# sayands/sgaligner

Measured on AMD Instinct MI355X. Metric: subscan-pairs/sec (fwd+bwd) + node-match Hits@1 vs reference, higher is better.
Workload: dtype f32 (fp32 operands and fp32 accumulation throughout; the anchors x negatives loss sweeps multiply them as three exact bf16 planes, six bf16 MFMAs per product...

## Files before the change

include/sgaligner_hip.h:

```cpp
#ifndef SGALIGNER_HIP_H
#define SGALIGNER_HIP_H
#include <stddef.h>
#include <stdint.h>
#ifdef __cplusplus
extern "C" {
#endif

int sga_version(void);
const char* sga_last_error(void);
int sga_device_cus(void);

int sga_pointnet_fwd(const float* x, const float* w1, const float* b1, const float* w2, const float* b2,
                     const float* w3, const float* b3, float* y, int32_t* argmax, int T, int P, int C3,
                     void* stream);
size_t sga_pointnet_fwd_ws_bytes(int T, int C3);
int sga_pointnet_fwd_ws(const float* x, const float* w1, const float* b1, const float* w2, const float* b2,
                        const float* w3, const float* b3, float* y, int32_t* argmax, int T, int P, int C3,
                        void* workspace, size_t ws_bytes, int mode, void* stream);
size_t sga_pointnet_fwd_bn_ws_bytes(int T, int C3);
int sga_pointnet_fwd_bn(const float* x, const float* w1, const float* b1, const float* w2, const float* b2,
                        const float* w3, const float* b3, float* y, int32_t* argmax, int T, int P, int C3,
                        void* workspace, size_t ws_bytes, void* bn_workspace, size_t bn_ws_bytes, double* bn_sums, int mode, void* stream);
int sga_pointnet_bwd(const float* x, const int32_t* argmax, const float* y, const float* gy, const float* w1,
                     const float* b1, const float* w2, const float* b2, const float* w3, float* gw1, float* gb1,
// ... 71 lines not shown
                      float* dZ, void* stream);
int sga_loss_neg_sums_shard(const float* Z, int Dp, int A, int J1, int J2, float tau0, float tau1, double* sums8, int a_lo, int a_hi,
                            void* stream);
int sga_loss_neg_grad_shard(const float* Z, int Dp, int A, int J1, int J2, float tau0, float tau1, const double* gs8,
                            float* dZ, int a_lo, int a_hi, void* stream);
size_t sga_loss_anchor_f16_ws_bytes(int NT, int A, int ns);
int sga_loss_anchor_fwd_f16(const float* const* Z, const void* const* Zh, const int* Dp, int NT, int A, const double* sums,
                            float alpha, float tau_icl, float tau_ial, double* out, int a_lo, int a_hi, void* ws, size_t ws_bytes,
                            void* stream);
int sga_loss_anchor_bwd_f16(const float* const* Z, const void* const* Zh, const int* Dp, int NT, int A, const double* sums,
                            float alpha, float tau_icl, float tau_ial, const float* coef, float* const* M1,
                            double* gs, int a_lo, int a_hi, void* ws, size_t ws_bytes, void* stream);

int sga_loss_stash_grad(const float* M1, const float* Z, int A, int Dp, float* dZ, int a_lo, int a_hi, void* stream);
int sga_loss_multi_sums(const float* const* Z, int M, int D, const float* beta, int A, int J1, int J2, float tau0, float tau1,
                        double* sums, int a_lo, int a_hi, void* stream);
int sga_loss_multi_grad(const float* const* Z, int M, int D, const float* beta, int A, int J1, int J2, float tau0, float tau1,
                        const double* gs, float* const* dZ, double* gamma, int a_lo, int a_hi, void* stream);
size_t sga_loss_centre_bytes(void);
int sga_loss_centre_tables(const float* Z, int A, int J1, int J2, float* Zc, void* stat_ws, void* stream);
int sga_loss_multi_sums_centred(const float* const* Zc, int M, const float* beta, int A, int J1, int J2, float tau0, float tau1,
                                double* sums, int a_lo, int a_hi, void* stream);
int sga_loss_multi_grad_centred(const float* const* Zc, int M, const float* beta, int A, int J1, int J2, float tau0, float tau1,
                                const double* gs, float* const* dZ, double* gamma, int a_lo, int a_hi, void* stream);
int sga_loss_scatter_tangent_stat(const float* dZ, const float* Z, const float* nrm, const int32_t* idx, int R, int D,
                                  const void* stat_ws, float* dE, void* stream);
int sga_loss_anchor_multi_fwd(const float* const* Z, int M, const float* beta, int A, const double* sums, float alpha,
                              float tau_icl, float tau_ial, double* out, int a_lo, int a_hi, void* stream);
int sga_loss_anchor_multi_bwd(const float* const* Z, int M, const float* beta, int A, const double* sums, float alpha,
                              float tau_icl, float tau_ial, const float* coef, float* const* M1, double* gs, double* gamma,
                              int a_lo, int a_hi, double* out_terms, void* stream);
int sga_loss_anchor_multi_bwd_symx(const float* const* Z, int M, const float* beta, int A, const double* sums, float alpha,
                                   float tau_icl, float tau_ial, const float* coef, float* const* M1, float* const* M2,
                                   double* gs, double* gamma, int a_lo, int a_hi, int j_lo, int j_hi, int mir, double* out_terms, void* stream);
int sga_loss_stash_grad_symx(const float* M1, const float* M2, const float* Z, int A, int Dp, float* dZ, int a_lo, int a_hi,
                             int j_lo, int j_hi, int mir, void* stream);

int sga_loss_check_norms(const float* nrm, int n, float* poison, void* stream);

size_t sga_loss_split3_bytes(int A, int J1, int J2);
int sga_loss_split3_tables(const float* Z, int A, int J1, int J2, void* Zb, float* Zc, void* stream);
int sga_loss_multi_sums_bf16x6(const void* const* Zb, int M, const float* beta, int A, int J1, int J2, float tau0, float tau1,
                               double* sums, int a_lo, int a_hi, int lite, void* stream);
int sga_loss_multi_grad_bf16x6(const void* const* Zb, int M, const float* beta, int A, int J1, int J2, float tau0, float tau1,
                               const double* gs, float* const* dZ, double* gamma, int a_lo, int a_hi, void* stream);
int sga_loss_scatter_tangent(const float* dZ, const float* Z, const float* nrm, const int32_t* idx, int A, int J1, int J2, int D,
                             const void* Zb, float* dE, void* stream);
int sga_loss_stash_grad_symx_bf16x6(const float* M1, const float* M2, const void* Zb, int A, int J1, int J2, float* dZ,
                                    int a_lo, int a_hi, int j_lo, int j_hi, int mir, void* stream);
int sga_loss_anchor_multi_bwd_symx_bf16x6(const void* const* Zb, int M, const float* beta, int A, int J1, int J2, const double* sums,
                                          float alpha, float tau_icl, float tau_ial, const float* coef, float* const* M1, float* const* M2,
                                          double* gs, double* gamma, int a_lo, int a_hi, int j_lo, int j_hi, int mir, double* out_terms,
                                          void* stream);

int sga_group_loss_fwd(const float* const* Z, int M, const float* beta, int A, int J1, const int32_t* groups, int G,
                       const int64_t* s_off, int64_t s_total, float alpha, float tau_icl, float tau_ial, float* S,
                       double* sums, double* out, int use_valu, void* stream);
int sga_group_loss_bwd(const float* const* Z, int M, const float* beta, int A, int J1, const int32_t* groups, int G,
                       const int64_t* s_off, int64_t s_total, float alpha, float tau_icl, float tau_ial, float* S,
                       const double* sums, const float* coef, float* const* dZ, double* gamma, int use_valu, void* stream);

size_t sga_simrank_workspace_bytes(int T);
size_t sga_simrank_workspace_bytes_f16(int T, int D);
int sga_simrank(const float* E, int T, int D, const int32_t* pair_off, const int32_t* blk_pair, const int32_t* blk_row, int n_blocks, int B,
                int max_pair_objects, const int32_t* q_idx, const int32_t* q_tgt, int Q, int K, int32_t* rank,
                int32_t* topk_idx, float* topk_sim, int f16, void* workspace, size_t workspace_bytes, void* stream);
int sga_pair_metrics(const int32_t* rank, const int32_t* topk_idx, const float* topk_sim, int K, const int32_t* q_tgt,
                     const int32_t* pair_off, const int32_t* pair_q_off, int B, float* out, void* stream);

int sga_gemm_ex(int transA, int transB, int M, int N, int K, const float* A, long lda, const float* B, long ldb,
                float* C, long ldc, const float* bias, int act, const float* resid, long ldr, void* stream);
int sga_pct_attention(const float* Q, long ldq, const float* V, long ldv, int T, int N, float* stats, float* Xs,
                      long ldx, void* stream);
int sga_pct_attention_bwd(const float* Q, long ldq, const float* V, long ldv, const float* dXs, long ldd, int T, int N,
                          const float* stats, float* work, float* dQ, long ldo, float* dV, long ldw, void* stream);
int sga_segment_max(const float* Y, long ldy, int T, int N, int C, float* G, int32_t* argmax, void* stream);
int sga_segment_max_bwd(const float* dG, const int32_t* argmax, int T, int N, int C, float* dY, long ldd, void* stream);
int sga_pct_head_prep(const float* dG, const float* G, const float* gamma, const float* beta, const float* fin, int T, int C, long R,
                      int training, float slope, float* coef, float* ab, void* stream);
int sga_pct_head_dw(const float* WG, const float* W, const float* ab, const float* cs, const float* coef, const int32_t* amax,
                    const float* cat, long ldc, int T, int N, int C, int K, float* dW, float* Wb, float* a0, void* stream);
int sga_pct_head_scatter(const float* coef, const int32_t* amax, const float* W, int T, int N, int C, int K, float* dcat, long ldd,
                         void* stream);
int sga_segment_max_affine(const float* Y, long ldy, int T, int N, int C, const float* scale, const float* shift, float slope, float* G,
                           int32_t* argmax, void* stream);

int sga_bn_stats(const float* X, long ldx, int R, int C, double* sums, void* stream);
int sga_bn_finalize(const double* sums, int R, int C, const float* gamma, const float* beta, float* running_mean, float* running_var,
                    long long* num_batches_tracked, float momentum, float eps, int training, float* out, void* stream);
int sga_bn_bwd_finalize(const double* sums, int R, int C, float* out, void* stream);
int sga_bn_apply(const float* X, long ldx, int R, int C, const float* scale, const float* shift, int act,
                 const float* resid, long ldr, float* Y, long ldy, void* stream);
int sga_bn_bwd_stats(const float* X, long ldx, const float* dY, long ldd, int R, int C, const float* scale,
                     const float* shift, const float* mean, const float* rstd, int act, double* sums, void* stream);
int sga_bn_bwd_apply(const float* X, long ldx, const float* dY, long ldd, int R, int C, const float* scale,
                     const float* shift, const float* mean, const float* rstd, const float* mean_g,
                     const float* mean_gx, int act, float* dX, long ldo, void* stream);

size_t sga_fps_scratch_floats(int total_points);
int sga_fps(const float* pts, const int32_t* offsets, int n_obj, const int32_t* start, int npoint,
            const int32_t* work_small, int n_small, const int32_t* work_mid, int n_mid,
            const int32_t* work_large, int n_large, int32_t* out_idx, float* scratch, void* stream);

int sga_hull_candidates(const float* pts, const int32_t* offsets, int n_obj, unsigned char* keep, int32_t* n_planes, void* stream);
int sga_hull_max_candidates(void);
int sga_hull_vertices(const double* pts, const int32_t* offsets, int n_obj, unsigned char* is_vertex, int32_t* status, void* stream);
// ... 70 lines not shown
```

sgaligner_amd/_lib.py:

```python
from __future__ import annotations

import ctypes
import os
from ctypes import c_char_p, c_double, c_float, c_int, c_int64, c_long, c_size_t, c_void_p

_HERE = os.path.dirname(os.path.abspath(__file__))
LIB_PATH = os.environ.get('SGA_LIB_PATH') or os.path.join(_HERE, 'csrc', 'libsga_hip.so')
_lib = None

P = c_void_p
I = c_int
F = c_float

SIGNATURES = {
    'sga_version': (I, []),
    'sga_last_error': (c_char_p, []),
    'sga_device_cus': (I, []),
    'sga_pointnet_fwd': (I, [P, P, P, P, P, P, P, P, P, I, I, I, P]),
    'sga_pointnet_fwd_ws_bytes': (c_size_t, [I, I]),
    'sga_loss_neg_grad_wide_floats': (c_size_t, [I, I, I]),
    'sga_loss_neg_grad_wide': (I, [P, I, I, I, I, c_float, c_float, P, P, P, c_size_t, P]),
    'sga_wide16_ldt': (c_long, [I, I, I]),
    'sga_wide16_prepare': (I, [P, I, I, I, I, P, P, P]),
    'sga_loss_neg_sums_f16': (I, [P, I, I, I, I, c_float, c_float, P, I, I, P]),
# ... 38 lines not shown
    'sga_hull_max_candidates': (I, []),
    'sga_hull_vertices': (I, [P, P, I, P, P, P]),
    'sga_nn_workspace_bytes': (c_size_t, [I, I, I]),
    'sga_nn_search': (I, [P, P, I, I, P, I, P, I, I, I, I, P, P, I, P, P, P, c_size_t, P]),
    'sga_ransac_workspace_bytes': (c_size_t, [I, I, I, I]),
    'sga_ransac_rigid': (I, [P, P, I, I, P, P, I, I, I, I, P, P, c_double, I, P, P, P, P, P, P, P, c_size_t, P]),
    'sga_subscan_lds_slots': (I, []),
    'sga_frame_visibility': (I, [P, P, P, P, P, P, I, I, I, c_int64, I, I, P, P, P, P, P]),
    'sga_subscan_walk': (I, [P, P, P, P, P, P, I, I, I, c_int64, P, P, P, P, P, P, P, P]),
    'sga_subscan_object_counts': (I, [P, P, P, P, I, I, I, c_int64, I, P, I, P, I, P, P, P, P, P, P]),
    'sga_scenegraph_lds_slots': (I, []),
    'sga_scenegraph_tile': (I, []),
    'sga_graph_max_nodes': (I, []),
    'sga_object_counts': (I, [P, P, P, I, I, I, I, P, P, P, P]),
    'sga_object_partition_ws_bytes': (c_size_t, [I, I, I]),
    'sga_object_partition': (I, [P, P, P, P, P, I, I, I, I, I, I, P, P, P, P, P, P, P, c_size_t, P]),
    'sga_graph_complete': (I, [P, P, P, P, I, P, P, I, I, P, P, P, P, P, P, P, P, P, P]),
    'sga_bow_counts': (I, [P, P, I, I, I, P, P, P, P]),
    'sga_gemm': (I, [I, I, I, I, I, P, c_long, I, P, c_long, P, c_long, P, I, P]),
    'sga_colsum': (I, [P, c_long, I, I, P, I, P]),
    'sga_gemm_bnstats': (I, [I, I, I, P, c_long, P, c_long, P, c_long, P, P, P]),
    'sga_cast_f64_f32': (I, [P, P, c_size_t, P]),
    'sga_gemm_plan': (I, [I, I, I, I, I, c_long, c_long, c_long, c_long] + [I] * 9 + [P, P, P]),
    'sga_loss_gather': (I, [P, I, I, P, I, P, I, P, P]),
    'sga_loss_scatter': (I, [P, P, P, P, I, I, I, P, P]),
    'sga_loss_neg_sums': (I, [P, I, I, I, I, F, F, P, P]),
    'sga_loss_neg_grad': (I, [P, I, I, I, I, F, F, P, P, P]),
    'sga_loss_neg_sums_shard': (I, [P, I, I, I, I, F, F, P, I, I, P]),
    'sga_loss_neg_grad_shard': (I, [P, I, I, I, I, F, F, P, P, I, I, P]),
    'sga_loss_anchor_f16_ws_bytes': (c_size_t, [I, I, I]),
    'sga_loss_anchor_fwd_f16': (I, [P, P, P, I, I, P, F, F, F, P, I, I, P, c_size_t, P]),
    'sga_loss_anchor_bwd_f16': (I, [P, P, P, I, I, P, F, F, F, P, P, P, I, I, P, c_size_t, P]),
    'sga_loss_stash_grad_f16_bytes': (c_size_t, [I, I]),
    'sga_loss_stash_grad_f16': (I, [P, P, I, I, I, I, P, I, I, P, c_size_t, P]),
    'sga_loss_multi_sums': (I, [P, I, I, P, I, I, I, F, F, P, I, I, P]),
    'sga_loss_multi_grad': (I, [P, I, I, P, I, I, I, F, F, P, P, P, I, I, P]),
    'sga_loss_centre_bytes': (c_size_t, []),
    'sga_loss_centre_tables': (I, [P, I, I, I, P, P, P]),
    'sga_loss_multi_sums_centred': (I, [P, I, P, I, I, I, F, F, P, I, I, P]),
    'sga_loss_multi_grad_centred': (I, [P, I, P, I, I, I, F, F, P, P, P, I, I, P]),
    'sga_loss_scatter_tangent_stat': (I, [P, P, P, P, I, I, P, P, P]),
    'sga_loss_check_norms': (I, [P, I, P, P]),
    'sga_loss_slots': (I, []),
    'sga_loss_anchor_multi_fwd': (I, [P, I, P, I, P, F, F, F, P, I, I, P]),
    'sga_loss_anchor_multi_bwd': (I, [P, I, P, I, P, F, F, F, P, P, P, P, I, I, P, P]),
    'sga_loss_stash_grad': (I, [P, P, I, I, P, I, I, P]),
    'sga_loss_anchor_multi_bwd_symx': (I, [P, I, P, I, P, F, F, F, P, P, P, P, P, I, I, I, I, I, P, P]),
    'sga_loss_stash_grad_symx': (I, [P, P, P, I, I, P, I, I, I, I, I, P]),
    'sga_loss_split3_bytes': (c_size_t, [I, I, I]),
    'sga_loss_split3_tables': (I, [P, I, I, I, P, P, P]),
    'sga_loss_scatter_tangent': (I, [P, P, P, P, I, I, I, I, P, P, P]),
    'sga_loss_stash_grad_symx_bf16x6': (I, [P, P, P, I, I, I, P, I, I, I, I, I, P]),
    'sga_loss_anchor_multi_bwd_symx_bf16x6': (I, [P, I, P, I, I, I, P, F, F, F, P, P, P, P, P, I, I, I, I, I, P, P]),
    'sga_loss_multi_sums_bf16x6': (I, [P, I, P, I, I, I, F, F, P, I, I, I, P]),
    'sga_loss_multi_grad_bf16x6': (I, [P, I, P, I, I, I, F, F, P, P, P, I, I, P]),
    'sga_group_loss_fwd': (I, [P, I, P, I, I, P, I, P, c_int64, F, F, F, P, P, P, I, P]),
    'sga_group_loss_bwd': (I, [P, I, P, I, I, P, I, P, c_int64, F, F, F, P, P, P, P, P, I, P]),
    'sga_fusion_fwd': (I, [P, I, P, P, I, I, P]),
    'sga_fusion_bwd_workspace_bytes': (c_size_t, [I]),
    'sga_fusion_bwd': (I, [P, I, P, P, P, P, I, I, P, c_size_t, P]),
    'sga_fusion_var_fwd': (I, [P, I, P, P, P, I, P]),
    'sga_fusion_var_bwd': (I, [P, I, P, P, P, P, P, I, P, c_size_t, P]),
    'sga_gcn_aggregate': (I, [P, I, P, P, P, P, I, I, I, I, P, P, P]),
    'sga_relu_bwd': (I, [P, P, P, c_size_t, P]),
    'sga_nca_row_group': (I, []),
    'sga_nca_block_sums': (I, [P, c_long, I, I, I, F, F, P, P, P, P]),
    'sga_nca_loss': (I, [P, P, I, P, I, F, F, P, P, P, P, P]),
    'sga_nca_coef': (I, [P, c_long, P, c_long, P, c_long, I, I, I, F, F, F, P, P, P, P]),
}

GEMM_ROUTES = ('EMPTY', 'TN_NARROW', 'TN_SPLIT', 'TN_BIG', 'NN', 'NT_128', 'NT_64', 'NT3_128', 'NT3_64', 'SMALL_F32', 'SMALL_F64',
               'GENERIC_F32', 'GENERIC_F64', 'REFUSED')


class SgaLibraryError(RuntimeError):
    pass


def lib():
    global _lib
    if _lib is None:
        if not os.path.exists(LIB_PATH):
            raise SgaLibraryError(
                f'HIP library not built: {LIB_PATH} is missing. Run `python -c "import __graft_entry__ as g; g.build()"` '
                f'(or `python -m sgaligner_amd._build`). sgaligner_amd has no CPU fallback.')
        import torch
        try:
            l = ctypes.CDLL(LIB_PATH)
        except OSError as e:
            raise SgaLibraryError(f'cannot load {LIB_PATH}: {e}') from e
        for name, (res, args) in SIGNATURES.items():
            try:
                fn = getattr(l, name)
            except AttributeError as e:
                raise SgaLibraryError(f'{LIB_PATH} does not export {name}; rebuild the library') from e
            fn.restype = res
            fn.argtypes = args
        _lib = l
    return _lib


def check(rc: int, what: str):
    if rc != 0:
        msg = lib().sga_last_error()
        raise RuntimeError(f'{what} failed (code {rc}): {msg.decode() if msg else "?"}')
```

sgaligner_amd/csrc/aa_epilogue.h:

```cpp
#pragma once
#include "loss_math.h"

namespace {

struct AnchorMultiArgs {
    int M, A, i_lo, i_hi, nsplit;
    const float* Z[4];
    const float* beta;
    const double* sums;
    const float* inv;
    float alpha, kc, ki, itc, iti;
    double* out;
    const float* coef;
    float* M1[4];
    double* gs;
    double* gamma;
    int j_lo;
    float* M2[4];
    int j_hi, mir;
};

__global__ void inv_sums_kernel(const double* __restrict__ sums, float* __restrict__ inv, int n) {
    const int i = blockIdx.x * blockDim.x + threadIdx.x;
    if (i < n) inv[i] = (float)(1.0 / (sums[i] + 1e-9));
}

template <int M, bool TERMS>
__device__ __forceinline__ void aa_flush(const AnchorMultiArgs& a, const float* inv_s, const int lane, const int slot,
                                         float (&acc_gs)[M + 1][8], float (&acc_gam)[M], float (&acc_out)[TERMS ? 3 * M + 1 : 1]) {
    constexpr int NT = M + 1;
    if (TERMS) {
#pragma unroll
        for (int e = 0; e < NT + 2 * M; ++e) {
            const float v = wave_sum(acc_out[TERMS ? e : 0]);
            if (lane == 0 && v != 0.f) atomicAdd(a.out + (NT + 2 * M) * (1 + slot) + e, (double)v);
            acc_out[TERMS ? e : 0] = 0.f;
        }
    }
#pragma unroll
    for (int k = 0; k < NT; ++k)
#pragma unroll
        for (int e = 0; e < 8; ++e) {
            const float iv2 = inv_s[k * 8 + e];
            const float v = -iv2 * iv2 * wave_sum(acc_gs[k][e]);
            if (lane == 0 && v != 0.f) atomicAdd(a.gs + NT * 8 * (1 + slot) + k * 8 + e, (double)v);
            acc_gs[k][e] = 0.f;
        }
#pragma unroll
    for (int m = 0; m < M; ++m) {
        const float v = wave_sum(acc_gam[m]);
        if (lane == 0 && v != 0.f) atomicAdd(a.gamma + M * (1 + slot) + m, (double)v);
        acc_gam[m] = 0.f;
    }
}

template <int M, bool TERMS, bool MASKED>
__device__ __forceinline__ void aa_epilogue(const AnchorMultiArgs& a, const float* inv_s, const float (&beta)[M], const f32x4 (&P)[M],
                                            const f32x4 (&Q)[M], float (&acc_gs)[M + 1][8], float (&acc_gam)[M], float (&acc_out)[TERMS ? 3 * M + 1 : 1],
                                            const int jg, const int JH, const bool iv, const int my_i, const int ns) {
    constexpr int NT = M + 1;
    auto CF = [&](int e) { return a.coef[e]; };
    const float* js = inv_s + M * 8;
    const float cJ = CF(M);
#pragma unroll
    for (int r = 0; r < 4; ++r) {
        const int j = jg + r;
        const bool ok = !MASKED || (iv && (j < JH));
        const float okf = (!MASKED || ok) ? 1.f : 0.f;
        float xj = 0.f, yj = 0.f;
#pragma unroll
        for (int m = 0; m < M; ++m) { xj = fmaf(beta[m], P[m][r], xj); yj = fmaf(beta[m], Q[m][r], yj); }
        float gJ, EA = 0.f, EB = 0.f;
        {
// ... 160 lines not shown
```

sgaligner_amd/csrc/aa_launch.h:

```cpp
#pragma once
#include "aa_epilogue.h"

namespace {

enum AAWalk {
    AA_ORDERED,
    AA_SYMMETRIC,
    AA_EITHER
};

struct AAContract {
    const char* name;
    int m_lo, m_hi;
    int row_align;
    int col_tile;
    AAWalk walk;
};

struct AAOperands {
    const void* const* tables;
    int M; const float* beta; int A; const double* sums;
    float alpha, tau_icl, tau_ial;
    const float* coef; float* const* M1; float* const* M2; double *gs, *gamma;
    int a_lo, a_hi, j_lo, j_hi, mir;
    double* out_terms;
};

template <class KArgs>
struct AAKernels {
    void (*sym)(KArgs), (*terms)(KArgs), (*plain)(KArgs);
    int rows;
    int shares;
    size_t lds;
};

static float* aa_inv_block(double* gs, int M) { return reinterpret_cast<float*>(gs + (size_t)(1 + SGA_SLOTS) * (M + 1) * 8); }

static int aa_plan(int nib, int ntile, int shares, int rounds) {
    int nsp = (rounds * sga_num_cus() + nib - 1) / nib;
    if (nsp > (ntile + shares - 1) / shares) nsp = (ntile + shares - 1) / shares;
    return nsp < 1 ? 1 : nsp;
}

static void aa_fill(AnchorMultiArgs& a, int M, const float* beta, int A, const double* sums, float alpha, float tau_icl, float tau_ial, int a_lo, int a_hi) {
    a.M = M; a.A = A; a.i_lo = a_lo; a.i_hi = a_hi; a.beta = beta; a.sums = sums; a.alpha = alpha;
    a.kc = LOG2E / tau_icl; a.ki = LOG2E / tau_ial; a.itc = 1.f / tau_icl; a.iti = 1.f / tau_ial;
}

static bool aa_symmetric(const AAContract& c, const AAOperands& o) {
    return c.walk == AA_SYMMETRIC || (c.walk == AA_EITHER && !(o.j_lo == 0 && o.j_hi == o.A && o.mir >= o.j_hi));
}

static int aa_validate(const AAContract& c, const AAOperands& o) {
    const int A = o.A, ra = c.row_align, ct = c.col_tile;
    SGA_CHECK_ARG(o.tables && o.beta && o.sums && o.coef && o.M1 && o.gs && o.gamma && A >= 0, "%s: bad argument", c.name);
    SGA_CHECK_ARG(o.M >= c.m_lo && o.M <= c.m_hi, "%s: M=%d not in %d..%d tables", c.name, o.M, c.m_lo, c.m_hi);
    SGA_CHECK_ARG(o.a_lo >= 0 && o.a_lo <= o.a_hi && o.a_hi <= A && o.a_lo % ra == 0 && (o.a_hi % ra == 0 || o.a_hi == A),
                  "%s: block [%d,%d) not on %d-row boundaries of [0,%d]", c.name, o.a_lo, o.a_hi, ra, A);
    SGA_CHECK_ARG(o.j_lo >= 0 && o.j_lo % ct == 0 && o.j_hi <= A && o.j_lo <= o.j_hi && (o.j_hi % ct == 0 || o.j_hi == A) && o.mir >= o.j_lo &&
                      (o.mir % ct == 0 || o.mir >= o.j_hi),
                  "%s: columns [%d,%d) / mirror start %d not on %d-column boundaries", c.name, o.j_lo, o.j_hi, o.mir, ct);
    if (aa_symmetric(c, o)) {
        SGA_CHECK_ARG(o.mir <= o.j_lo || (o.j_lo >= o.a_lo && (o.mir < o.j_hi ? o.mir : o.j_hi) <= o.a_hi),
                      "%s: ordered columns [%d,%d) outside the block's square [%d,%d)", c.name, o.j_lo, o.mir, o.a_lo, o.a_hi);
        SGA_CHECK_ARG(o.out_terms, "%s: a symmetric launch returns its terms (out_terms == NULL)", c.name);
    }
    for (int m = 0; m < o.M; ++m)
        SGA_CHECK_ARG(o.tables[m] && o.M1[m] && (o.mir >= o.j_hi || (o.M2 && o.M2[m])), "%s: null table or stash", c.name);
    return SGA_OK;
}

template <class KArgs>
static int aa_run(const AAContract& c, const AAOperands& o, KArgs& k, AnchorMultiArgs& a, const AAKernels<KArgs>& kern, int threads, int rounds,
                  void* stream) {
    hipStream_t s = static_cast<hipStream_t>(stream);
    const int M = o.M, NT = M + 1;
    if (int rc = zero_slots(o.gs, NT * 8, s, c.name)) return rc;
    if (int rc = zero_slots(o.gamma, M, s, c.name)) return rc;
    if (o.out_terms) { if (int rc = zero_slots(o.out_terms, NT + 2 * M, s, c.name)) return rc; }
    if (o.A == 0 || o.a_hi <= o.a_lo || o.j_hi <= o.j_lo) return SGA_OK;
    aa_fill(a, M, o.beta, o.A, o.sums, o.alpha, o.tau_icl, o.tau_ial, o.a_lo, o.a_hi);
    a.coef = o.coef; a.gs = o.gs; a.gamma = o.gamma; a.out = o.out_terms;
    a.j_lo = o.j_lo; a.j_hi = o.j_hi; a.mir = o.mir;
    for (int m = 0; m < M; ++m) { a.M1[m] = o.M1[m]; a.M2[m] = o.M2 ? o.M2[m] : nullptr; }
    float* inv = aa_inv_block(o.gs, M);
    hipLaunchKernelGGL(inv_sums_kernel, dim3(1), dim3(64), 0, s, o.sums, inv, NT * 8);
    a.inv = inv;
    const int nib = (o.a_hi - o.a_lo + kern.rows - 1) / kern.rows, ntile16 = ((o.j_hi + c.col_tile - 1) / c.col_tile * c.col_tile - o.j_lo) / 16;
    a.nsplit = aa_plan(nib, ntile16, kern.shares, rounds);
    auto fn = aa_symmetric(c, o) ? kern.sym : o.out_terms ? kern.terms : kern.plain;
    hipFuncSetAttribute(reinterpret_cast<const void*>(fn), hipFuncAttributeMaxDynamicSharedMemorySize, (int)kern.lds);
    hipLaunchKernelGGL(fn, dim3(nib * a.nsplit), dim3(threads), kern.lds, s, k);
    if (o.out_terms) fold_slots(o.out_terms, NT + 2 * M, s);
    fold_slots(o.gs, NT * 8, s);
    fold_slots(o.gamma, M, s);
    SGA_CHECK_LAUNCH(c.name);
    return SGA_OK;
}

}
```

sgaligner_amd/csrc/anchor3.hip:

```cpp
#include "mfma_tiles.h"
#include <type_traits>

#include "s3_layout.h"
#include "aa_launch.h"

namespace {

constexpr int A3_THREADS = 512;
constexpr int A3_TW = 4;
constexpr int A3_NOP = 11;
constexpr size_t a3_lds_bytes(int M) { return (size_t)M * 2 * 2 * A3_NOP * 1024; }
static_assert(a3_lds_bytes(3) <= 160 * 1024, "the own rows of three tables fit a CU's LDS");

struct Anchor3Args {
    AnchorMultiArgs a;
    const unsigned char* Zb[4];
    int nbA;
};

__device__ __forceinline__ u32x4 a3_ld(const unsigned char* p) { return *reinterpret_cast<const u32x4*>(p); }

template <int M, bool TERMS, bool SYM>
__global__ __launch_bounds__(A3_THREADS) void anchor3_bwd_kernel(Anchor3Args A3) {
    static_assert(!SYM || TERMS, "symmetric mode: one-pass build");
    static_assert(M == 2 || M == 3, "two or three tables");
    const AnchorMultiArgs& a = A3.a;
    extern __shared__ __attribute__((aligned(16))) u32x4 own3[];
    const float* __restrict__ inv_s = a.inv;
    const int tid = threadIdx.x, lane = tid & 63, wave = tid >> 6, g = lane >> 4, l15 = lane & 15;
    const int A = a.A, ns = a.i_hi - a.i_lo;
    const int JH = SYM ? a.j_hi : A;
    const int ib = blockIdx.x / a.nsplit, split = blockIdx.x % a.nsplit;
    const int i0 = a.i_lo + ib * 32;
    const int ih = wave & 1, tw = wave >> 1;
    const int my_i = i0 + ih * 16 + l15;
    const bool iv = my_i < a.i_hi;

    if (tid < 256) {
        const int ln = tid & 63, hh = (tid >> 6) & 1, side = tid >> 7;
        const int gg = ln >> 4, o = hh * 16 + (ln & 15);
        const int ojh = (o >> 2) & 1, oi = 4 * (o >> 3) + (o & 3);
        const int so = (ojh * 64 + s3_slot(gg, oi)) * 16;
#pragma unroll
        for (int m = 0; m < M; ++m) {
            const unsigned char* base = A3.Zb[m] + (size_t)(side * A3.nbA + (i0 >> 5)) * S3_BLOCK;
            u32x4* dst = own3 + (((m * 2 + side) * 2 + hh) * A3_NOP) * 64 + ln;
            const unsigned char* tb = base + S3_TAIL + ojh * 1024;
            const u32x4 th = a3_ld(tb + s3_slot(0, oi) * 16), tm = a3_ld(tb + s3_slot(2, oi) * 16), tl = a3_ld(tb + s3_slot(3, oi) * 16);
            u32x4 ot[2];
            s3_own_tails(th, tm, tl, gg, ot);
            dst[0] = ot[1];
            dst[64] = ot[0];
#pragma unroll
            for (int p = 0; p < 3; ++p)
#pragma unroll
                for (int q = 0; q < 3; ++q) dst[(2 + p * 3 + q) * 64] = a3_ld(base + p * S3_PLANE + q * 2048 + so);
        }
    }
    __syncthreads();
    float beta[M];
#pragma unroll
    for (int m = 0; m < M; ++m) beta[m] = a.beta[m];

    constexpr int NT = M + 1;
    float acc_gs[NT][8], acc_gam[M];
#pragma unroll
    for (int k = 0; k < NT; ++k)
#pragma unroll
        for (int e = 0; e < 8; ++e) acc_gs[k][e] = 0.f;
#pragma unroll
    for (int m = 0; m < M; ++m) acc_gam[m] = 0.f;
    float acc_out[TERMS ? NT + 2 * M : 1];
#pragma unroll
    for (int e = 0; e < (TERMS ? NT + 2 * M : 1); ++e) acc_out[e] = 0.f;
    int tiles_done = 0;
    const int slot = my_slot();

    const int aoff = s3_slot(g, l15) * 16;
    const int jt_end = 2 * ((JH + 31) >> 5);
#pragma unroll 1
    for (int jt = (a.j_lo >> 4) + split * A3_TW + tw; jt < jt_end; jt += a.nsplit * A3_TW) {
        const int jb = jt >> 1, jh = jt & 1, j0 = 32 * jb;
        int lofs = 0;
        asm volatile("" : "+v"(lofs));
        f32x4 P[M], Q[M];
        struct JF { u32x4 t, p[3][3]; };
        auto jload = [&](int ss, JF& o) {
            const unsigned char* ar = A3.Zb[ss >> 1] + (size_t)(((ss & 1) ? 0 : A3.nbA) + jb) * S3_BLOCK + jh * 1024 + aoff;
            o.t = a3_ld(ar + S3_TAIL);
#pragma unroll
            for (int p = 0; p < 3; ++p)
#pragma unroll
                for (int q = 0; q < 3; ++q) o.p[p][q] = a3_ld(ar + p * S3_PLANE + q * 2048);
        };
        JF jf[2];
        jload(0, jf[0]);
#pragma unroll
        for (int ss = 0; ss < 2 * M; ++ss) {
            if (ss + 1 < 2 * M) jload(ss + 1, jf[(ss + 1) & 1]);
            __builtin_amdgcn_sched_barrier(0);
            const JF& o = jf[ss & 1];
            const u32x4* bo = own3 + lofs + ((ss * 2 + ih) * A3_NOP) * 64 + lane;
            u32x4 ow[A3_NOP];
#pragma unroll
            for (int k = 0; k < A3_NOP; ++k) ow[k] = bo[k * 64];
            constexpr int PA[6] = {2, 1, 1, 0, 0, 0}, PB[6] = {0, 1, 0, 2, 1, 0};
            f32x4 acc = f32x4{0.f, 0.f, 0.f, 0.f};
            acc = mfma_b(o.t, ow[0], acc);
            acc = mfma_b(o.t, ow[1], acc);
#pragma unroll
            for (int x = 0; x < 6; ++x)
#pragma unroll
                for (int q = 0; q < 3; ++q) acc = mfma_b(o.p[PA[x]][q], ow[2 + PB[x] * 3 + q], acc);
            if (ss & 1) Q[ss >> 1] = acc; else P[ss >> 1] = acc;
            __builtin_amdgcn_sched_barrier(0);
        }
        const int jg = j0 + 8 * g + 4 * jh;
        if constexpr (SYM) {
            if (j0 >= a.mir) aa_epilogue_sym<M>(a, inv_s, beta, P, Q, acc_gs, acc_gam, acc_out, jg, JH, iv, my_i, ns);
            else aa_epilogue<M, TERMS, true>(a, inv_s, beta, P, Q, acc_gs, acc_gam, acc_out, jg, JH, iv, my_i, ns);
        } else {
            if (j0 + 32 <= A && i0 + 32 <= a.i_hi) aa_epilogue<M, TERMS, false>(a, inv_s, beta, P, Q, acc_gs, acc_gam, acc_out, jg, JH, iv, my_i, ns);
            else aa_epilogue<M, TERMS, true>(a, inv_s, beta, P, Q, acc_gs, acc_gam, acc_out, jg, JH, iv, my_i, ns);
        }
        if ((++tiles_done & (SYM ? 15 : 31)) == 0) aa_flush<M, TERMS>(a, inv_s, lane, slot, acc_gs, acc_gam, acc_out);
    }
    aa_flush<M, TERMS>(a, inv_s, lane, slot, acc_gs, acc_gam, acc_out);
}

template <int M>
AAKernels<Anchor3Args> anchor3_kernels() {
    return {anchor3_bwd_kernel<M, true, true>, anchor3_bwd_kernel<M, true, false>, anchor3_bwd_kernel<M, false, false>, 32, A3_TW, a3_lds_bytes(M)};
}

}

extern "C" int sga_loss_anchor_multi_bwd_symx_bf16x6(const void* const* Zb, int M, const float* beta, int A, int J1, int J2, const double* sums,
                                                     float alpha, float tau_icl, float tau_ial, const float* coef, float* const* M1, float* const* M2,
                                                     double* gs, double* gamma, int a_lo, int a_hi, int j_lo, int j_hi, int mir, double* out_terms,
                                                     void* stream) {
    static const AAContract C = {"sga_loss_anchor_multi_bwd_symx_bf16x6", 2, 3, 32, 32, AA_EITHER};
    const AAOperands o = {Zb, M, beta, A, sums, alpha, tau_icl, tau_ial, coef, M1, M2, gs, gamma, a_lo, a_hi, j_lo, j_hi, mir, out_terms};
    SGA_CHECK_ARG(J1 >= 0 && J2 >= 0, "sga_loss_anchor_multi_bwd_symx_bf16x6: bad argument");
    if (int rc = aa_validate(C, o)) return rc;
    Anchor3Args k{};
    k.nbA = make_tlayout(A, J1, J2).nbA;
    for (int m = 0; m < M; ++m) k.Zb[m] = static_cast<const unsigned char*>(Zb[m]);
    return aa_run(C, o, k, k.a, M == 2 ? anchor3_kernels<2>() : anchor3_kernels<3>(), A3_THREADS, 3, stream);
}
```

sgaligner_amd/csrc/loss_anchor.hip:

```cpp
#include "mfma_tiles.h"
#include <type_traits>

#include "loss_math.h"
#include "aa_launch.h"

extern "C" int sga_gemm(int transA, int transB, int M, int N, int K, const void* A, long lda, int a_is_f64, const float* B,
                        long ldb, float* C, long ldc, const float* bias, int accumulate, void* stream);

namespace {

constexpr int CT_THREADS = 256;
template <int M>
__global__ __launch_bounds__(CT_THREADS, M <= 3 ? 2 : 1) void anchor_multi_kernel(AnchorMultiArgs a) {
    constexpr int DP = 104, NQ = 13, NT = M + 1;
    extern __shared__ __attribute__((aligned(16))) float lds[];
    float* inv_s = lds + M * 2 * 32 * DP;
    const int tid = threadIdx.x, lane = tid & 63, wave = tid >> 6, h = lane >> 5, l31 = lane & 31;
    const int A = a.A, ns = a.i_hi - a.i_lo;
    const int ib = blockIdx.x / a.nsplit, split = blockIdx.x % a.nsplit;
    const int i0 = a.i_lo + ib * 32;
    const int my_i = i0 + l31;
    const bool iv = my_i < a.i_hi;

    for (int e = tid; e < M * 2 * 32 * (DP / 4); e += CT_THREADS) {
// ... 52 lines not shown
        const float* js = inv_s + M * 8;
#pragma unroll
        for (int r = 0; r < 16; ++r) {
            const int j = j0 + mfma32_row(r, h);
            const bool ok = iv && j < A;
            float xj = 0.f, yj = 0.f;
#pragma unroll
            for (int m = 0; m < M; ++m) { xj = fmaf(beta[m], xs[m][r], xj); yj = fmaf(beta[m], ys[m][r], yj); }
            {
                const float dji = fexp2(xj * a.ki);
                const float qma = g_val(dji, js[1], js[3]), qmb = g_val(dji, js[5], js[7]);
                const float lqma = flog(qma), lqmb = flog(qmb);
#pragma unroll
                for (int k = 0; k < NT; ++k) {
                    const float x = k < M ? xs[k < M ? k : 0][r] : xj, y = k < M ? ys[k < M ? k : 0][r] : yj;
                    const float* is = inv_s + k * 8;
                    const float qa = g_val(fexp2(x * a.kc), is[0], is[2]);
                    const float qb = g_val(fexp2(y * a.kc), is[4], is[6]);
                    const float term = -flog(a.alpha * qa + (1.f - a.alpha) * qb);
                    acc_out[k] += ok ? term : 0.f;
                    if (k < M) {
                        const float dm = fexp2(x * a.ki);
                        const float qoa = g_val(dm, is[1], is[3]), qob = g_val(dm, is[5], is[7]);
                        const float ta = __expf(qoa) * (qoa - lqma), tb = __expf(qob) * (qob - lqmb);
                        acc_out[NT + (k < M ? k : 0)] += ok ? ta : 0.f;
                        acc_out[NT + M + (k < M ? k : 0)] += ok ? tb : 0.f;
                    }
                }
            }
#pragma unroll
            for (int e = 0; e < NT + 2 * M; ++e) asm volatile("" : "+v"(acc_out[e]));
            __builtin_amdgcn_sched_barrier(0);
        }
#pragma unroll
        for (int e = 0; e < NT + 2 * M; ++e) acc_d[e] += (double)acc_out[e];
    }
    const int slot = my_slot();
#pragma unroll
    for (int e = 0; e < NT + 2 * M; ++e) {
        const double v = wave_sum_d(acc_d[e]);
        if (lane == 0 && v != 0.0) atomicAdd(a.out + (NT + 2 * M) * (1 + slot) + e, v);
    }
}

template <int M, bool TERMS = false, int RB = (M <= 3 ? 32 : 16), bool SYM = false>
__global__ __launch_bounds__(CT_THREADS, 2) void anchor_multi_bwd16_kernel(AnchorMultiArgs a) {
    static_assert(!SYM || TERMS, "symmetric mode: one-pass build");
    constexpr int DP = 104, NT = M + 1, NSUB = RB / 16, TW = 4 / NSUB;
    extern __shared__ __attribute__((aligned(16))) float lds[];
    const float* __restrict__ inv_s = a.inv;
    const int tid = threadIdx.x, lane = tid & 63, wave = tid >> 6, g = lane >> 4, l15 = lane & 15;
    const int A = a.A, ns = a.i_hi - a.i_lo;
    const int JH = SYM ? a.j_hi : A;
    const int ib = blockIdx.x / a.nsplit, split = blockIdx.x % a.nsplit;
    const int i0 = a.i_lo + ib * RB;
    const int ih = wave % NSUB, tw = wave / NSUB;
    const int my_i = i0 + ih * 16 + l15;
    const bool iv = my_i < a.i_hi;

    for (int e = tid; e < M * 2 * RB * (DP / 4); e += CT_THREADS) {
        const int c = (e % (DP / 4)) * 4, r = (e / (DP / 4)) % RB, side = (e / (DP / 4) / RB) % 2, m = e / (DP / 4) / (2 * RB);
        const int row = min(i0 + r, a.i_hi - 1) + side * A;
        *reinterpret_cast<f32x4*>(lds + ((m * 2 + side) * RB + r) * DP + c) = *reinterpret_cast<const f32x4*>(a.Z[m] + (size_t)row * DP + c);
    }
    __syncthreads();
    float beta[M];
#pragma unroll
    for (int m = 0; m < M; ++m) beta[m] = a.beta[m];

    float acc_gs[NT][8], acc_gam[M];
#pragma unroll
    for (int k = 0; k < NT; ++k)
#pragma unroll
        for (int e = 0; e < 8; ++e) acc_gs[k][e] = 0.f;
#pragma unroll
    for (int m = 0; m < M; ++m) acc_gam[m] = 0.f;
    float acc_out[TERMS ? NT + 2 * M : 1];
#pragma unroll
    for (int e = 0; e < (TERMS ? NT + 2 * M : 1); ++e) acc_out[e] = 0.f;
    int tiles_done = 0;
    const int slot = my_slot();
    auto flush = [&]() { aa_flush<M, TERMS>(a, inv_s, lane, slot, acc_gs, acc_gam, acc_out); };

    const int ntile = (JH + 15) / 16;
#pragma unroll 1
    for (int jt = (a.j_lo >> 4) + split * TW + tw; jt < ntile; jt += a.nsplit * TW) {
        const int j0 = jt * 16;
        const int jrow = min(j0 + l15, A - 1);
        int lofs = 0;
        asm volatile("" : "+v"(lofs));
        f32x4 P[M], Q[M];
        struct JOps { f32x4 p[6], q[6]; float pt[2], qt[2]; };
        auto jload = [&](int m, JOps& o) {
            const float* gp = a.Z[m] + (size_t)(A + jrow) * DP;
            const float* gq = a.Z[m] + (size_t)jrow * DP;
#pragma unroll
            for (int q = 0; q < 6; ++q) {
                o.p[q] = *reinterpret_cast<const f32x4*>(gp + 16 * q + 4 * g);
                o.q[q] = *reinterpret_cast<const f32x4*>(gq + 16 * q + 4 * g);
            }
#pragma unroll
            for (int t = 0; t < 2; ++t) { o.pt[t] = gp[96 + 4 * t + g]; o.qt[t] = gq[96 + 4 * t + g]; }
        };
        constexpr bool JDB = true;
        JOps jb[JDB ? 2 : 1];
        jload(0, jb[0]);
#pragma unroll
        for (int m = 0; m < M; ++m) {
            if (JDB) { if (m + 1 < M) jload(m + 1, jb[JDB ? (m + 1) & 1 : 0]); }
            else if (m > 0) jload(m, jb[0]);
            __builtin_amdgcn_sched_barrier(0);
            P[m] = f32x4{0.f, 0.f, 0.f, 0.f};
            Q[m] = P[m];
            const JOps& o = jb[JDB ? m & 1 : 0];
            const float* bp = lds + lofs + ((m * 2 + 0) * RB + ih * 16 + l15) * DP;
            const float* bq = lds + lofs + ((m * 2 + 1) * RB + ih * 16 + l15) * DP;
#pragma unroll
            for (int q = 0; q < 6; ++q) {
                const f32x4 b1 = *reinterpret_cast<const f32x4*>(bp + 16 * q + 4 * g);
                const f32x4 b2 = *reinterpret_cast<const f32x4*>(bq + 16 * q + 4 * g);
#pragma unroll
                for (int r = 0; r < 4; ++r) {
                    P[m] = __builtin_amdgcn_mfma_f32_16x16x4f32(o.p[q][r], b1[r], P[m], 0, 0, 0);
                    Q[m] = __builtin_amdgcn_mfma_f32_16x16x4f32(o.q[q][r], b2[r], Q[m], 0, 0, 0);
                }
            }
#pragma unroll
            for (int t = 0; t < 2; ++t) {
                const int kk = 96 + 4 * t + g;
                P[m] = __builtin_amdgcn_mfma_f32_16x16x4f32(o.pt[t], bp[kk], P[m], 0, 0, 0);
                Q[m] = __builtin_amdgcn_mfma_f32_16x16x4f32(o.qt[t], bq[kk], Q[m], 0, 0, 0);
            }
            __builtin_amdgcn_sched_barrier(0);
        }
        const int jg = j0 + 4 * g;
        if constexpr (SYM) {
            if (j0 >= a.mir) aa_epilogue_sym<M>(a, inv_s, beta, P, Q, acc_gs, acc_gam, acc_out, jg, JH, iv, my_i, ns);
            else aa_epilogue<M, TERMS, true>(a, inv_s, beta, P, Q, acc_gs, acc_gam, acc_out, jg, JH, iv, my_i, ns);
        } else {
            if (j0 + 16 <= A && i0 + RB <= a.i_hi) aa_epilogue<M, TERMS, false>(a, inv_s, beta, P, Q, acc_gs, acc_gam, acc_out, jg, JH, iv, my_i, ns);
            else aa_epilogue<M, TERMS, true>(a, inv_s, beta, P, Q, acc_gs, acc_gam, acc_out, jg, JH, iv, my_i, ns);
        }
        if ((++tiles_done & (SYM ? 15 : 31)) == 0) flush();
    }
    flush();
}

}

extern "C" int sga_loss_anchor_multi_fwd(const float* const* Z, int M, const float* beta, int A, const double* sums,
                                         float alpha, float tau_icl, float tau_ial, double* out, int a_lo, int a_hi,
                                         void* stream) {
    SGA_CHECK_ARG(Z && beta && sums && out && A >= 0, "sga_loss_anchor_multi_fwd: bad argument");
    SGA_CHECK_ARG(M >= 2 && M <= 4, "sga_loss_anchor_multi_fwd: M=%d not in {2,3,4} (use the per-table kernels)", M);
    SGA_CHECK_ARG(a_lo >= 0 && a_hi <= A && a_lo <= a_hi, "sga_loss_anchor_multi_fwd: anchor shard [%d,%d) outside [0,%d]", a_lo, a_hi, A);
    for (int m = 0; m < M; ++m) SGA_CHECK_ARG(Z[m], "sga_loss_anchor_multi_fwd: null table");
    hipStream_t s = static_cast<hipStream_t>(stream);
    const int n = (M + 1) + 2 * M;
    if (int rc0 = zero_slots(out, n, s, "sga_loss_anchor_multi_fwd")) return rc0;
    if (A == 0 || a_hi <= a_lo) return SGA_OK;
    AnchorMultiArgs a{};
    aa_fill(a, M, beta, A, sums, alpha, tau_icl, tau_ial, a_lo, a_hi);
    for (int m = 0; m < M; ++m) a.Z[m] = Z[m];
    a.out = out;
    const int nib = (a_hi - a_lo + 31) / 32;
    a.nsplit = aa_plan(nib, (A + 31) / 32, 4, 4);
    const size_t lds = (size_t)(M * 2 * 32 * 104 + (M + 1) * 8) * sizeof(float);
    auto k = M == 2 ? anchor_multi_kernel<2> : M == 3 ? anchor_multi_kernel<3> : anchor_multi_kernel<4>;
    hipFuncSetAttribute(reinterpret_cast<const void*>(k), hipFuncAttributeMaxDynamicSharedMemorySize, (int)lds);
    hipLaunchKernelGGL(k, dim3(nib * a.nsplit), dim3(CT_THREADS), lds, s, a);
    fold_slots(out, n, s);
    SGA_CHECK_LAUNCH("sga_loss_anchor_multi_fwd");
    return SGA_OK;
}

template <int M>
static AAKernels<AnchorMultiArgs> anchor_multi_bwd_kernels() {
    constexpr int RB = M <= 3 ? 32 : 16;
    return {anchor_multi_bwd16_kernel<M, true, RB, true>, anchor_multi_bwd16_kernel<M, true>, anchor_multi_bwd16_kernel<M, false>, RB, 64 / RB,
            (size_t)(M * 2 * RB * 104 + (M + 1) * 8) * sizeof(float)};
}

static int anchor_multi_bwd(const AAContract& c, const AAOperands& o, const float* const* Z, void* stream) {
    if (int rc = aa_validate(c, o)) return rc;
    AnchorMultiArgs a{};
    for (int m = 0; m < o.M; ++m) a.Z[m] = Z[m];
    const auto kern = o.M == 2 ? anchor_multi_bwd_kernels<2>() : o.M == 3 ? anchor_multi_bwd_kernels<3>() : anchor_multi_bwd_kernels<4>();
    return aa_run(c, o, a, a, kern, CT_THREADS, 6, stream);
}

extern "C" int sga_loss_anchor_multi_bwd(const float* const* Z, int M, const float* beta, int A, const double* sums,
                                         float alpha, float tau_icl, float tau_ial, const float* coef, float* const* M1,
                                         double* gs, double* gamma, int a_lo, int a_hi, double* out_terms, void* stream) {
    static const AAContract C = {"sga_loss_anchor_multi_bwd", 2, 4, 1, 16, AA_ORDERED};
    return anchor_multi_bwd(C, {reinterpret_cast<const void* const*>(Z), M, beta, A, sums, alpha, tau_icl, tau_ial, coef, M1, nullptr, gs, gamma,
                                a_lo, a_hi, 0, A, A, out_terms}, Z, stream);
}

extern "C" int sga_loss_anchor_multi_bwd_symx(const float* const* Z, int M, const float* beta, int A, const double* sums, float alpha,
                                              float tau_icl, float tau_ial, const float* coef, float* const* M1, float* const* M2,
                                              double* gs, double* gamma, int a_lo, int a_hi, int j_lo, int j_hi, int mir, double* out_terms,
                                              void* stream) {
    static const AAContract C = {"sga_loss_anchor_multi_bwd_symx", 2, 4, 32, 16, AA_SYMMETRIC};
    return anchor_multi_bwd(C, {reinterpret_cast<const void* const*>(Z), M, beta, A, sums, alpha, tau_icl, tau_ial, coef, M1, M2, gs, gamma,
                                a_lo, a_hi, j_lo, j_hi, mir, out_terms}, Z, stream);
}

extern "C" int sga_loss_stash_grad_symx(const float* M1, const float* M2, const float* Z, int A, int Dp, float* dZ, int a_lo, int a_hi,
                                        int j_lo, int j_hi, int mir, void* stream) {
    SGA_CHECK_ARG(M1 && Z && dZ && A >= 0 && Dp >= 8 && Dp % 8 == 0 && a_lo >= 0 && a_hi <= A && a_lo <= a_hi && j_lo >= 0 && j_lo <= j_hi && j_hi <= A &&
                  mir >= j_lo && (M2 || mir >= j_hi), "sga_loss_stash_grad_symx: bad argument");
    const int ns = a_hi - a_lo, c1 = j_hi - j_lo, c2 = mir < j_hi ? j_hi - mir : 0;
    if (A == 0 || ns == 0 || c1 == 0) return SGA_OK;
    const float* X1 = Z;
    const float* X2 = Z + (size_t)A * Dp;
    float* d1 = dZ;
    float* d2 = dZ + (size_t)A * Dp;
    int rc = sga_gemm(1, 0, ns, Dp, c1, M1, ns, 0, X2 + (size_t)j_lo * Dp, Dp, d1 + (size_t)a_lo * Dp, Dp, nullptr, 1, stream);
    if (!rc) rc = sga_gemm(0, 0, c1, Dp, ns, M1, ns, 0, X1 + (size_t)a_lo * Dp, Dp, d2 + (size_t)j_lo * Dp, Dp, nullptr, 1, stream);
    if (!rc && c2 > 0) rc = sga_gemm(0, 0, c2, Dp, ns, M2, ns, 0, X2 + (size_t)a_lo * Dp, Dp, d1 + (size_t)mir * Dp, Dp, nullptr, 1, stream);
    if (!rc && c2 > 0) rc = sga_gemm(1, 0, ns, Dp, c2, M2, ns, 0, X1 + (size_t)mir * Dp, Dp, d2 + (size_t)a_lo * Dp, Dp, nullptr, 1, stream);
    return rc;
}
```

Before: 1001.

## Plan anchor-loss grid with occupancy-aware two-run split to balance wave tails

Replaces the fixed anchor-loss work split (rounds × CU count / row blocks) with a planner. The planner queries real per-CU occupancy and searches split counts, allowing two groups of row blocks with different column-split factors, to minimise estimated wave rounds and tail imbalance. Kernels decode their block id into (row block, split, stride) through the new helper. It adds a cached occupancy query and a plan-inspection entry point, at the risk of a cost model that picks worse grids for some shapes.

Result: faster. 1019, median of 6 (+1.8%).

```diff
diff --git a/include/sgaligner_hip.h b/include/sgaligner_hip.h
--- a/include/sgaligner_hip.h
+++ b/include/sgaligner_hip.h
@@ -147,6 +147,7 @@
                                           float alpha, float tau_icl, float tau_ial, const float* coef, float* const* M1, float* const* M2,
                                           double* gs, double* gamma, int a_lo, int a_hi, int j_lo, int j_hi, int mir, double* out_terms,
                                           void* stream);
+int sga_loss_anchor_plan(int planes, int M, int A, int a_lo, int a_hi, int j_lo, int j_hi, int slots, int32_t* plan);
 
 int sga_group_loss_fwd(const float* const* Z, int M, const float* beta, int A, int J1, const int32_t* groups, int G,
                        const int64_t* s_off, int64_t s_total, float alpha, float tau_icl, float tau_ial, float* S,
diff --git a/sgaligner_amd/_lib.py b/sgaligner_amd/_lib.py
--- a/sgaligner_amd/_lib.py
+++ b/sgaligner_amd/_lib.py
@@ -114,6 +114,7 @@
     'sga_loss_scatter_tangent': (I, [P, P, P, P, I, I, I, I, P, P, P]),
     'sga_loss_stash_grad_symx_bf16x6': (I, [P, P, P, I, I, I, P, I, I, I, I, I, P]),
     'sga_loss_anchor_multi_bwd_symx_bf16x6': (I, [P, I, P, I, I, I, P, F, F, F, P, P, P, P, P, I, I, I, I, I, P, P]),
+    'sga_loss_anchor_plan': (I, [I, I, I, I, I, I, I, I, P]),
     'sga_loss_multi_sums_bf16x6': (I, [P, I, P, I, I, I, F, F, P, I, I, I, P]),
     'sga_loss_multi_grad_bf16x6': (I, [P, I, P, I, I, I, F, F, P, P, P, I, I, P]),
     'sga_group_loss_fwd': (I, [P, I, P, I, I, P, I, P, c_int64, F, F, F, P, P, P, I, P]),
diff --git a/sgaligner_amd/csrc/aa_epilogue.h b/sgaligner_amd/csrc/aa_epilogue.h
--- a/sgaligner_amd/csrc/aa_epilogue.h
+++ b/sgaligner_amd/csrc/aa_epilogue.h
@@ -18,7 +18,14 @@
     int j_lo;
     float* M2[4];
     int j_hi, mir;
+    int nib1, nsplit2;
 };
+
+__device__ __forceinline__ void aa_unit(const AnchorMultiArgs& a, int& ib, int& split, int& ns) {
+    const int b = blockIdx.x, n1 = a.nib1 * a.nsplit;
+    if (b < n1) { ns = a.nsplit; ib = b / ns; split = b - ib * ns; }
+    else { ns = a.nsplit2; ib = (b - n1) / ns; split = (b - n1) - ib * ns; ib += a.nib1; }
+}
 
 __global__ void inv_sums_kernel(const double* __restrict__ sums, float* __restrict__ inv, int n) {
     const int i = blockIdx.x * blockDim.x + threadIdx.x;
diff --git a/sgaligner_amd/csrc/aa_launch.h b/sgaligner_amd/csrc/aa_launch.h
--- a/sgaligner_amd/csrc/aa_launch.h
+++ b/sgaligner_amd/csrc/aa_launch.h
@@ -1,4 +1,7 @@
 #pragma once
+#include <algorithm>
+#include <mutex>
+
 #include "aa_epilogue.h"
 
 namespace {
@@ -26,20 +29,69 @@
     double* out_terms;
 };
 
+struct AAGeom {
+    int rows;
+    int shares;
+    int col_tile;
+    int rounds;
+};
+
 template <class KArgs>
 struct AAKernels {
     void (*sym)(KArgs), (*terms)(KArgs), (*plain)(KArgs);
-    int rows;
-    int shares;
+    AAGeom g;
     size_t lds;
 };
 
 static float* aa_inv_block(double* gs, int M) { return reinterpret_cast<float*>(gs + (size_t)(1 + SGA_SLOTS) * (M + 1) * 8); }
 
-static int aa_plan(int nib, int ntile, int shares, int rounds) {
-    int nsp = (rounds * sga_num_cus() + nib - 1) / nib;
-    if (nsp > (ntile + shares - 1) / shares) nsp = (ntile + shares - 1) / shares;
-    return nsp < 1 ? 1 : nsp;
+constexpr AAGeom aa_geom(bool planes, int M) { return planes ? AAGeom{32, 4, 32, 1} : M <= 3 ? AAGeom{32, 2, 16, 3} : AAGeom{16, 4, 16, 3}; }
+
+struct AAPlan { int nib1, n1, n2, wgs; long long cost; };
+
+static AAPlan aa_plan(int nib, int ntile, int shares, int slots, int rounds, bool two_runs = true) {
+    const int steps = (ntile + shares - 1) / shares, cap = steps < 1 ? 1 : steps;
+    if (slots < 1) slots = 1;
+    if (nib < 1) return {0, 1, 1, 0, 0};
+    auto cdiv = [](long long a, long long b) { return (a + b - 1) / b; };
+    const int want = (int)cdiv((long long)rounds * slots, nib);
+    const int lo1 = std::min(want, cap), hi1 = std::min(lo1 + 15, cap), hi2 = two_runs ? std::min(cap, std::max(hi1, 64)) : 0;
+    AAPlan best = {0, 1, 1, 0, -1};
+    auto take = [&](int nib1, int n1, int n2, long long cost) {
+        const int wgs = nib1 * n1 + (nib - nib1) * n2;
+        if (best.cost < 0 || cost < best.cost || (cost == best.cost && wgs < best.wgs)) best = {nib1, n1, n2, wgs, cost};
+    };
+    for (int n1 = lo1; n1 <= hi1; ++n1) {
+        const long long c1 = cdiv(steps, n1) + 1;
+        take(nib, n1, n1, cdiv((long long)nib * n1, slots) * c1);
+        const long long F = (long long)nib * n1 / slots;
+        const int nib1 = (int)(F * slots / n1);
+        if (nib1 >= nib) continue;
+        for (int n2 = 1; n2 <= hi2; ++n2) take(nib1, n1, n2, F * c1 + cdiv((long long)(nib - nib1) * n2, slots) * (cdiv(steps, n2) + 1));
+    }
+    return best;
+}
+
+static AAPlan aa_job_plan(const AAGeom& g, int a_lo, int a_hi, int j_lo, int j_hi, int slots) {
+    const int nib = (a_hi - a_lo + g.rows - 1) / g.rows, ntile16 = ((j_hi + g.col_tile - 1) / g.col_tile * g.col_tile - j_lo) / 16;
+    return aa_plan(nib, ntile16, g.shares, slots, g.rounds);
+}
+
+static int aa_slots(const void* fn, int threads, size_t lds) {
+    struct Seen { const void* fn; int dev, per_cu; };
+    constexpr int NSEEN = 32;
+    static Seen seen[NSEEN];
+    static int nseen = 0;
+    static std::mutex mu;
+    int dev = 0;
+    if (hipGetDevice(&dev) != hipSuccess) { (void)hipGetLastError(); dev = 0; }
+    std::lock_guard<std::mutex> lock(mu);
+    for (int i = 0; i < nseen; ++i)
+        if (seen[i].fn == fn && seen[i].dev == dev) return seen[i].per_cu * sga_num_cus();
+    int per_cu = 0;
+    if (hipOccupancyMaxActiveBlocksPerMultiprocessor(&per_cu, fn, threads, lds) != hipSuccess || per_cu < 1) { (void)hipGetLastError(); per_cu = 1; }
+    if (nseen < NSEEN) seen[nseen++] = {fn, dev, per_cu};
+    return per_cu * sga_num_cus();
 }
 
 static void aa_fill(AnchorMultiArgs& a, int M, const float* beta, int A, const double* sums, float alpha, float tau_icl, float tau_ial, int a_lo, int a_hi) {
@@ -71,8 +123,7 @@
 }
 
 template <class KArgs>
-static int aa_run(const AAContract& c, const AAOperands& o, KArgs& k, AnchorMultiArgs& a, const AAKernels<KArgs>& kern, int threads, int rounds,
-                  void* stream) {
+static int aa_run(const AAContract& c, const AAOperands& o, KArgs& k, AnchorMultiArgs& a, const AAKernels<KArgs>& kern, int threads, void* stream) {
     hipStream_t s = static_cast<hipStream_t>(stream);
     const int M = o.M, NT = M + 1;
     if (int rc = zero_slots(o.gs, NT * 8, s, c.name)) return rc;
@@ -86,11 +137,11 @@
     float* inv = aa_inv_block(o.gs, M);
     hipLaunchKernelGGL(inv_sums_kernel, dim3(1), dim3(64), 0, s, o.sums, inv, NT * 8);
     a.inv = inv;
-    const int nib = (o.a_hi - o.a_lo + kern.rows - 1) / kern.rows, ntile16 = ((o.j_hi + c.col_tile - 1) / c.col_tile * c.col_tile - o.j_lo) / 16;
-    a.nsplit = aa_plan(nib, ntile16, kern.shares, rounds);
     auto fn = aa_symmetric(c, o) ? kern.sym : o.out_terms ? kern.terms : kern.plain;
     hipFuncSetAttribute(reinterpret_cast<const void*>(fn), hipFuncAttributeMaxDynamicSharedMemorySize, (int)kern.lds);
-    hipLaunchKernelGGL(fn, dim3(nib * a.nsplit), dim3(threads), kern.lds, s, k);
+    const AAPlan p = aa_job_plan(kern.g, o.a_lo, o.a_hi, o.j_lo, o.j_hi, aa_slots(reinterpret_cast<const void*>(fn), threads, kern.lds));
+    a.nib1 = p.nib1; a.nsplit = p.n1; a.nsplit2 = p.n2;
+    hipLaunchKernelGGL(fn, dim3(p.wgs), dim3(threads), kern.lds, s, k);
     if (o.out_terms) fold_slots(o.out_terms, NT + 2 * M, s);
     fold_slots(o.gs, NT * 8, s);
     fold_slots(o.gamma, M, s);
diff --git a/sgaligner_amd/csrc/anchor3.hip b/sgaligner_amd/csrc/anchor3.hip
--- a/sgaligner_amd/csrc/anchor3.hip
+++ b/sgaligner_amd/csrc/anchor3.hip
@@ -30,7 +30,8 @@
     const int tid = threadIdx.x, lane = tid & 63, wave = tid >> 6, g = lane >> 4, l15 = lane & 15;
     const int A = a.A, ns = a.i_hi - a.i_lo;
     const int JH = SYM ? a.j_hi : A;
-    const int ib = blockIdx.x / a.nsplit, split = blockIdx.x % a.nsplit;
+    int ib, split, nsp;
+    aa_unit(a, ib, split, nsp);
     const int i0 = a.i_lo + ib * 32;
     const int ih = wave & 1, tw = wave >> 1;
     const int my_i = i0 + ih * 16 + l15;
@@ -79,7 +80,7 @@
     const int aoff = s3_slot(g, l15) * 16;
     const int jt_end = 2 * ((JH + 31) >> 5);
 #pragma unroll 1
-    for (int jt = (a.j_lo >> 4) + split * A3_TW + tw; jt < jt_end; jt += a.nsplit * A3_TW) {
+    for (int jt = (a.j_lo >> 4) + split * A3_TW + tw; jt < jt_end; jt += nsp * A3_TW) {
         const int jb = jt >> 1, jh = jt & 1, j0 = 32 * jb;
         int lofs = 0;
         asm volatile("" : "+v"(lofs));
@@ -130,7 +131,8 @@
 
 template <int M>
 AAKernels<Anchor3Args> anchor3_kernels() {
-    return {anchor3_bwd_kernel<M, true, true>, anchor3_bwd_kernel<M, true, false>, anchor3_bwd_kernel<M, false, false>, 32, A3_TW, a3_lds_bytes(M)};
+    static_assert(aa_geom(true, M).rows == 32 && aa_geom(true, M).shares == A3_TW, "the plan's numbers are this kernel's");
+    return {anchor3_bwd_kernel<M, true, true>, anchor3_bwd_kernel<M, true, false>, anchor3_bwd_kernel<M, false, false>, aa_geom(true, M), a3_lds_bytes(M)};
 }
 
 }
@@ -146,5 +148,5 @@
     Anchor3Args k{};
     k.nbA = make_tlayout(A, J1, J2).nbA;
     for (int m = 0; m < M; ++m) k.Zb[m] = static_cast<const unsigned char*>(Zb[m]);
-    return aa_run(C, o, k, k.a, M == 2 ? anchor3_kernels<2>() : anchor3_kernels<3>(), A3_THREADS, 3, stream);
+    return aa_run(C, o, k, k.a, M == 2 ? anchor3_kernels<2>() : anchor3_kernels<3>(), A3_THREADS, stream);
 }
diff --git a/sgaligner_amd/csrc/loss_anchor.hip b/sgaligner_amd/csrc/loss_anchor.hip
--- a/sgaligner_amd/csrc/loss_anchor.hip
+++ b/sgaligner_amd/csrc/loss_anchor.hip
@@ -128,7 +128,8 @@
     const int tid = threadIdx.x, lane = tid & 63, wave = tid >> 6, g = lane >> 4, l15 = lane & 15;
     const int A = a.A, ns = a.i_hi - a.i_lo;
     const int JH = SYM ? a.j_hi : A;
-    const int ib = blockIdx.x / a.nsplit, split = blockIdx.x % a.nsplit;
+    int ib, split, nsp;
+    aa_unit(a, ib, split, nsp);
     const int i0 = a.i_lo + ib * RB;
     const int ih = wave % NSUB, tw = wave / NSUB;
     const int my_i = i0 + ih * 16 + l15;
@@ -160,7 +161,7 @@
 
     const int ntile = (JH + 15) / 16;
 #pragma unroll 1
-    for (int jt = (a.j_lo >> 4) + split * TW + tw; jt < ntile; jt += a.nsplit * TW) {
+    for (int jt = (a.j_lo >> 4) + split * TW + tw; jt < ntile; jt += nsp * TW) {
         const int j0 = jt * 16;
         const int jrow = min(j0 + l15, A - 1);
         int lofs = 0;
@@ -240,10 +241,10 @@
     for (int m = 0; m < M; ++m) a.Z[m] = Z[m];
     a.out = out;
     const int nib = (a_hi - a_lo + 31) / 32;
-    a.nsplit = aa_plan(nib, (A + 31) / 32, 4, 4);
     const size_t lds = (size_t)(M * 2 * 32 * 104 + (M + 1) * 8) * sizeof(float);
     auto k = M == 2 ? anchor_multi_kernel<2> : M == 3 ? anchor_multi_kernel<3> : anchor_multi_kernel<4>;
     hipFuncSetAttribute(reinterpret_cast<const void*>(k), hipFuncAttributeMaxDynamicSharedMemorySize, (int)lds);
+    a.nsplit = aa_plan(nib, (A + 31) / 32, 4, aa_slots(reinterpret_cast<const void*>(k), CT_THREADS, lds), 4, false).n1;
     hipLaunchKernelGGL(k, dim3(nib * a.nsplit), dim3(CT_THREADS), lds, s, a);
     fold_slots(out, n, s);
     SGA_CHECK_LAUNCH("sga_loss_anchor_multi_fwd");
@@ -253,7 +254,8 @@
 template <int M>
 static AAKernels<AnchorMultiArgs> anchor_multi_bwd_kernels() {
     constexpr int RB = M <= 3 ? 32 : 16;
-    return {anchor_multi_bwd16_kernel<M, true, RB, true>, anchor_multi_bwd16_kernel<M, true>, anchor_multi_bwd16_kernel<M, false>, RB, 64 / RB,
+    static_assert(aa_geom(false, M).rows == RB && aa_geom(false, M).shares == 64 / RB, "the plan's numbers are this kernel's");
+    return {anchor_multi_bwd16_kernel<M, true, RB, true>, anchor_multi_bwd16_kernel<M, true>, anchor_multi_bwd16_kernel<M, false>, aa_geom(false, M),
             (size_t)(M * 2 * RB * 104 + (M + 1) * 8) * sizeof(float)};
 }
 
@@ -262,7 +264,18 @@
     AnchorMultiArgs a{};
     for (int m = 0; m < o.M; ++m) a.Z[m] = Z[m];
     const auto kern = o.M == 2 ? anchor_multi_bwd_kernels<2>() : o.M == 3 ? anchor_multi_bwd_kernels<3>() : anchor_multi_bwd_kernels<4>();
-    return aa_run(c, o, a, a, kern, CT_THREADS, 6, stream);
+    return aa_run(c, o, a, a, kern, CT_THREADS, stream);
+}
+
+extern "C" int sga_loss_anchor_plan(int planes, int M, int A, int a_lo, int a_hi, int j_lo, int j_hi, int slots, int32_t* plan) {
+    SGA_CHECK_ARG(plan && slots >= 1 && M >= 2 && M <= (planes ? 3 : 4) && A >= 0 && a_lo >= 0 && a_lo <= a_hi && a_hi <= A && j_lo >= 0 && j_lo <= j_hi &&
+                      j_hi <= A && j_lo % 16 == 0, "sga_loss_anchor_plan: bad argument");
+    const AAGeom g = aa_geom(planes != 0, M);
+    const AAPlan p = aa_job_plan(g, a_lo, a_hi, j_lo, j_hi, slots);
+    const int nib = (a_hi - a_lo + g.rows - 1) / g.rows, ntile16 = ((j_hi + g.col_tile - 1) / g.col_tile * g.col_tile - j_lo) / 16;
+    const int32_t out[8] = {g.rows, g.shares, nib, p.nib1, p.n1, p.n2, j_hi > j_lo ? p.wgs : 0, (ntile16 + g.shares - 1) / g.shares};
+    for (int i = 0; i < 8; ++i) plan[i] = out[i];
+    return SGA_OK;
 }
 
 extern "C" int sga_loss_anchor_multi_bwd(const float* const* Z, int M, const float* beta, int A, const double* sums,
```
